# peterrum/dealii-multigrid

Measured on AMD Instinct MI355X. Metric: DoF/s per V-cycle, 3D octant p=4, higher is better.
Workload: dtype f64; 1 GPU; 3D octant (GeometryType quadrant) HMG-global p=4 FP64, NRefGlobal=8, SmootherDegree=3, coarse solver direct, f=1, zero Dirichlet (BASELINE.json configs[2]); n_dofs=137199985, n_cells=2127189, n_levels=9, parallelism=1 GPU, chebyshev_start_vector=deal.II's (i mod 11) - mean on the local numbering, fused_transfer_bricks=33509

## Files before the change

### dealii_multigrid_amd/csrc/kernels_apply.hpp

```cpp
#pragma once
#include "kernels_common.hpp"

namespace mgamd
{
#ifdef MGAMD_KERNEL_DEBUG
#define MGAMD_STAMP(k)                         \
  if (args.stamps && tid == 0)                 \
    args.stamps[(size_t)block * 8 + (k)] = wall_clock64();
#define MGAMD_ABLATED(bit) (args.ablate & (bit))
#else
#define MGAMD_STAMP(k)
#define MGAMD_ABLATED(bit) false
#endif

  template <typename T, int P>
  __device__ __forceinline__ void
  interior_diag_terms(const Mats<P, T> &mats, const int t, T &s_K, T &s_M)
  {
    const int tt[3] = {t % P, (t / P) % P, t / (P * P)};
    T         m[3], k[3];
#pragma unroll
    for (int d = 0; d < 3; ++d)
      {
        T dm = T(0), dk = T(0);
// ... 1174 lines not shown
#pragma unroll
          for (int a = 0; a <= P; ++a)
            {
              dM[c * P + a] += T(args.m.M[a * (P + 1) + a]);
              dK[c * P + a] += T(args.m.K[a * (P + 1) + a]);
            }
        const T sh3 = T(args.sigma) * q * h;
        T       mx = T(0), kx = T(0), my = T(0), ky = T(0);
#pragma unroll
        for (int i = 0; i < G::N; ++i)
          {
            if (i == u)
              {
                mx = dM[i];
                kx = dK[i];
              }
            if (i == v)
              {
                my = dM[i];
                ky = dK[i];
              }
          }
#pragma unroll
        for (int i = 0; i < G::N; ++i)
          bufD[sl * G::N3 + (i * G::N + v) * G::N + u] = h * (kx * my * dM[i] + mx * ky * dM[i] + mx * my * dK[i]) + sh3 * (mx * my * dM[i]);
      }
    __syncthreads();
    if (B == 1)
      {
        const bool any_hanging = __syncthreads_or((int)(mask >> 3)) != 0;
        if (any_hanging)
          for (int j = 0; j < G::N3; ++j)
            {
              for (int idx = tid; idx < G::SPW * G::N3; idx += G::BLOCK)
                bufA[idx] = (idx % G::N3) == j ? T(1) : T(0);
              __syncthreads();
              hanging_passes<T, P>(bufA, args.m, sl, u, v, act, mask, false);
              lattice_sweeps<T, P, B, G::BLOCK>(bufA, bufB, args.m, tid, nslots, args.g.h + slot0, NoHook(), false, args.sigma, args.g.q + slot0);
              hanging_passes<T, P>(bufA, args.m, sl, u, v, act, mask, true);
              if (act && ln == 0 && (mask >> 3))
                bufD[sl * G::N3 + j] = bufA[sl * G::N3 + j];
              __syncthreads();
            }
      }
    if constexpr (brick_may_be_constrained(B, CONSTR))
      {
        uint32_t fm = 0;
        if (args.g.fmask != nullptr && tid < nslots)
          fm = args.g.fmask[slot0 + tid];
        const bool any_family = __syncthreads_or((int)(fm != 0)) != 0;
        if (any_family)
          for (int s = 0; s < G::N_SHELL; ++s)
            {
              const int j = args.g.shell_pos[s];
              for (int idx = tid; idx < G::SPW * G::N3; idx += G::BLOCK)
                bufA[idx] = (idx % G::N3) == j ? T(1) : T(0);
              __syncthreads();
              brick_constraint_passes<T, P, B, G::BLOCK>(bufA, args.m, tid, nslots, args.g.fmask + slot0, false);
              lattice_sweeps<T, P, B, G::BLOCK>(bufA, bufB, args.m, tid, nslots, args.g.h + slot0, NoHook(), false, args.sigma, args.g.q + slot0);
              brick_constraint_passes<T, P, B, G::BLOCK>(bufA, args.m, tid, nslots, args.g.fmask + slot0, true);
              if (act && ln == 0 && args.g.fmask[slot0 + sl])
                bufD[sl * G::N3 + j] = bufA[sl * G::N3 + j];
              __syncthreads();
            }
      }
    if (G::N_INT > 0)
      for (int idx = tid; idx < nslots * G::N_INT; idx += G::BLOCK)
        {
          const int sl2 = idx / (G::N_INT > 0 ? G::N_INT : 1), i = idx % (G::N_INT > 0 ? G::N_INT : 1);
          const int x = i % (G::NI > 0 ? G::NI : 1), y = (i / (G::NI > 0 ? G::NI : 1)) % (G::NI > 0 ? G::NI : 1),
                    z = i / (G::NI > 0 ? G::NI * G::NI : 1);
          const T d = bufD[sl2 * G::N3 + ((z + 1) * G::N + (y + 1)) * G::N + x + 1];
          apply_epilogue<T, MODE_INVDIAG>(args.epi, args.g.interior_base[slot0 + sl2] + i, d);
        }
    for (int idx = tid; idx < nslots * G::N_SHELL; idx += G::BLOCK)
      {
        const int      sl2 = idx / G::N_SHELL, s = idx % G::N_SHELL;
        const uint32_t gi  = args.g.shell_idx[(size_t)(slot0 + sl2) * G::N_SHELL + s];
        if (gi < args.scatter_limit)
          atomic_add(&args.tail_acc[gi - args.n_interior], bufD[sl2 * G::N3 + args.g.shell_pos[s]]);
      }
  }

  template <typename T, int MODE_>
  __global__ void
  __launch_bounds__(256) tail_kernel(T *__restrict__ tail_acc, uint32_t n_interior, uint32_t n_tail, uint32_t n_rest, Epilogue<T> epi)
  {
    constexpr int  MODE   = base_mode(MODE_);
    constexpr bool FUSE_P = MODE_ == MODE_CHEB_PROLONGATE;
    constexpr int  U      = 4;
    const uint32_t total  = n_tail + n_rest;
    const uint32_t stride = gridDim.x * blockDim.x;
    __shared__ T   dtable[256];
    const bool     coded = is_cheb(MODE) && epi.dinv_code != nullptr;
    if (coded)
      {
        dtable[threadIdx.x] = epi.dinv_table[threadIdx.x];
        __syncthreads();
      }
    for (uint32_t i0 = blockIdx.x * blockDim.x + threadIdx.x; i0 < total; i0 += U * stride)
      {
        T ax[U], xv[U], xo[U], bv[U], dv[U];
#pragma unroll
        for (int u = 0; u < U; ++u)
          {
            const uint32_t i  = i0 + u * stride;
            const uint32_t gi = n_interior + i;
            ax[u] = xv[u] = xo[u] = bv[u] = dv[u] = T(0);
            if (i < total)
              {
                if (MODE != MODE_INVDIAG && MODE != MODE_CHEB_FIRST && MODE != MODE_MASS && (is_cheb(MODE) || i >= n_tail))
                  {
                    if (FUSE_P && i < n_tail && NT_LOAD(&epi.xs_flag[i]))
                      {
                        xv[u] = NT_LOAD(&epi.xs[gi]);
                        epi.x_inout[gi] = xv[u];
                      }
                    else
                      xv[u] = NT_LOAD(&epi.x[gi]);
                  }
                ax[u] = i < n_tail ? tail_acc[i] : xv[u];
                if (MODE == MODE_RESIDUAL || is_cheb(MODE))
                  bv[u] = NT_LOAD(&epi.b[gi]);
                if (is_cheb(MODE))
                  {
                    if (MODE == MODE_CHEB && epi.xold)
                      xo[u] = NT_LOAD(&epi.xold[gi]);
                    if (coded)
                      {
                        const uint32_t c = NT_LOAD(&epi.dinv_code[i]);
                        dv[u]            = c != 255u ? dtable[c] : epi.dinv[gi];
                      }
                    else
                      dv[u] = epi.dinv[gi];
                  }
              }
          }
#pragma unroll
        for (int u = 0; u < U; ++u)
          {
            const uint32_t i  = i0 + u * stride;
            const uint32_t gi = n_interior + i;
            if (i < total)
              {
                if (i < n_tail)
                  NT_STORE(T(0), &tail_acc[i]);
                if (MODE == MODE_CHEB_FIRST || MODE == MODE_CHEB_SECOND)
                  {
                    const T x1 = epi.c0 * dv[u] * bv[u];
                    if (MODE == MODE_CHEB_FIRST)
                      {
                        xv[u] = x1;
                        if (i >= n_tail)
                          ax[u] = x1;
                      }
                    else
                      xo[u] = x1;
                  }
                if (MODE == MODE_VMULT || MODE == MODE_MASS)
                  NT_STORE(ax[u], &epi.out[gi]);
                else if (MODE == MODE_RESIDUAL)
                  NT_STORE(bv[u] - ax[u], &epi.out[gi]);
                else if (is_cheb(MODE))
                  {
                    const T r = xv[u] + epi.f1 * (xv[u] - xo[u]) + epi.f2 * dv[u] * (bv[u] - ax[u]);
                    if (MODE_ == MODE_CHEB)
                      store_result(epi, gi, r);
                    else
                      NT_STORE(r, &epi.out[gi]);
                  }
                else
                  epi.out[gi] = (i < n_tail && fabs((double)ax[u]) > 1.0e-10) ? T(1) / ax[u] : T(1);
              }
          }
      }
  }

}
```

### dealii_multigrid_amd/csrc/level_operator.hpp

```cpp
#pragma once
#include "runtime.hpp"
#include "kernels.hpp"

#include <cmath>
#include <cstring>
#include <map>
#include <mutex>
#include <type_traits>
#include <unordered_map>

namespace mgamd
{
  inline int
  grid_for(size_t n)
  {
    size_t g = (n + 255) / 256;
    if (g > 2048)
      g = 2048;
    if (g < 1)
      g = 1;
    return (int)g;
  }

  template <typename T>
// ... 127 lines not shown
      if (any)
        h_cell.upload(g.h);
    }
    const double *
    scale(bool mass_pass) const
    {
      return mass_pass && h_cell.p ? h_cell.p : h.p;
    }
    SlotGroupDev
    view(bool mass_pass) const
    {
      return SlotGroupDev{interior_base.p, shell_idx.p, mask.p, scale(mass_pass), shell_pos.p, (uint32_t)n_slots, fmask.p, q.p};
    }
    SlotGroupDev
    view(size_t begin, size_t end, bool mass_pass) const
    {
      const size_t n_shell = (size_t)N * N * N - (size_t)(N - 2) * (N - 2) * (N - 2);
      return SlotGroupDev{interior_base.p + begin, shell_idx.p + begin * n_shell, mask.p + begin, scale(mass_pass) + begin, shell_pos.p,
                          (uint32_t)(end - begin), fmask.p ? fmask.p + begin : nullptr, q.p + begin};
    }
    DBuf<uint32_t> uniq_ptr, uniq_idx;
    DBuf<uint16_t> loc;
    uint32_t       max_uniq = 0;
    bool
    has_clusters() const
    {
      return uniq_ptr.p != nullptr;
    }
    CellClusterDev
    cluster_view(bool mass_pass) const
    {
      return CellClusterDev{uniq_ptr.p, uniq_idx.p, loc.p, mask.p, scale(mass_pass), (uint32_t)n_slots, max_uniq, q.p};
    }
    size_t
    cluster_lds_bytes() const
    {
      return 2 * (size_t)std::max<uint32_t>(max_uniq, 1) * sizeof(T);
    }
    void
    build_clusters(const SlotGroup &g)
    {
      const size_t          ns = g.n_slots(), ncl = (ns + CLUSTER_CELLS - 1) / CLUSTER_CELLS;
      std::vector<uint32_t> ptr(ncl + 1, 0), idx;
      std::vector<uint16_t> l(ns * 8, 0xFFFFu);
      std::vector<uint32_t> tmp;
      for (size_t c = 0; c < ncl; ++c)
        {
          const size_t s0 = c * CLUSTER_CELLS, s1 = std::min(ns, s0 + CLUSTER_CELLS);
          tmp.clear();
          for (size_t sl = s0; sl < s1; ++sl)
            for (int s = 0; s < 8; ++s)
              if (g.shell_idx[sl * 8 + s] != INVALID_DOF)
                tmp.push_back(g.shell_idx[sl * 8 + s]);
          std::sort(tmp.begin(), tmp.end());
          tmp.erase(std::unique(tmp.begin(), tmp.end()), tmp.end());
          for (size_t sl = s0; sl < s1; ++sl)
            for (int s = 0; s < 8; ++s)
              {
                const uint32_t gi = g.shell_idx[sl * 8 + s];
                if (gi != INVALID_DOF)
                  l[sl * 8 + g.shell_pos[s]] = (uint16_t)(std::lower_bound(tmp.begin(), tmp.end(), gi) - tmp.begin());
              }
          idx.insert(idx.end(), tmp.begin(), tmp.end());
          ptr[c + 1] = (uint32_t)idx.size();
          max_uniq   = std::max<uint32_t>(max_uniq, (uint32_t)tmp.size());
        }
      if (idx.empty())
        idx.push_back(0);
      uniq_ptr.upload(ptr);
      uniq_idx.upload(idx);
      loc.upload(l);
    }
  };

  template <typename T>
  struct FusedTransferHost
  {
    int                 group = -1;
    const uint32_t     *flags = nullptr;
    const uint32_t     *coarse_idx = nullptr;
    uint32_t            nc3 = 0;
    std::vector<double> E;
    const uint8_t      *tail_flags = nullptr;
    T *coarse = nullptr, *scratch = nullptr, *x_inout = nullptr;
  };
  constexpr bool
  fused_transfer_supported(int p)
  {
    return persistent_brick(p) != 0;
  }

  template <typename T>
  struct LevelOperator : LevelOperatorBase
  {
    int                                       p = 1;
    std::vector<std::unique_ptr<GroupDev<T>>> groups;
    DBuf<T>                                   tail_acc;
    DBuf<uint8_t>                             dinv_code;
    DBuf<T>                                   dinv_table;
    const T                                  *dinv_coded = nullptr;
    int                                       dominant_B = 0;
    uint32_t                                  ablate = 0;
    DBuf<unsigned long long>                  stamps;
    int                                       stamp_mode = -1;
    bool                                      halo_overlap = true;

    struct HaloDev
    {
      DBuf<uint32_t> pack_idx, sh_tail, sh_ptr;
      DBuf<int32_t>  sh_src, sh_owner_src;
      DBuf<T>        send, recv;
    };
    std::unique_ptr<HaloDev> halo;

    enum class LaunchKind
    {
      LATTICE,
      LATTICE_CONSTRAINED,
      BRICK_PAIR,
      BRICKS_AND_CELLS,
      BRICKS_AND_CLUSTERS,
      CLUSTERS
    };
    struct LaunchStep
    {
      LaunchKind   kind;
      GroupDev<T> *g, *partner;
      size_t       begin, end;
    };
    struct LaunchPlan
    {
      std::vector<LaunchStep> ordinary, diagonal;
      std::vector<LaunchStep> halo_slots, interior_slots;
    } plan;

    LevelOperator(Ctx *c, const mgamd_dofs *dofs, std::shared_ptr<Comm> cm)
    {
      ctx    = c;
      type   = (int)sizeof(T);
      tables = dofs->tables;
      tria   = dofs->tria;
      p      = tables->p;
      sigma  = tables->sigma;
      if (tables->ls_level && sigma != 0.0)
        throw std::invalid_argument("level operator: mass coefficient " + std::to_string(sigma) +
                                    " on a local-smoothing level: not implemented (refinement-edge matrices have no mass term)");
      if (cm && dofs->halo)
        {
          comm      = cm;
          halo_plan = dofs->halo;
          halo      = std::make_unique<HaloDev>();
          halo->pack_idx.upload(halo_plan->pack_idx);
          halo->sh_tail.upload(halo_plan->sh_tail);
          halo->sh_ptr.upload(halo_plan->sh_ptr);
          halo->sh_src.upload(halo_plan->sh_src);
          halo->sh_owner_src.upload(halo_plan->sh_owner_src);
          halo->send.alloc(std::max<size_t>(halo_plan->pack_idx.size(), 1));
          halo->recv.alloc(std::max<size_t>(halo_plan->pack_idx.size(), 1));
        }
      size_t best = 0;
      for (const SlotGroup &g : tables->groups)
        {
          auto d     = std::make_unique<GroupDev<T>>();
          d->B           = g.B;
          d->N           = g.N;
          d->constrained = g.constrained_group;
// ... 295 lines not shown
    void
    launch_bricks_and_cells(hipStream_t st, const ApplyArgs<T, P> &a, const GroupDev<T> &g1)
    {
      using G2 = Geo<P, 2>;
      SmallSlotsArgs<T, P> sa;
      sa.a           = a;
      sa.g_cells     = g1.view(MODE == MODE_MASS);
      sa.n_wg_bricks = (uint32_t)((a.g.n_slots + G2::SPW - 1) / G2::SPW);
      using GW = Geo<P, 1, 64>;
      const uint32_t n_w        = (uint32_t)((g1.n_slots + GW::SPW - 1) / GW::SPW);
      const uint32_t n_wg_cells = (n_w + CELL_WAVES - 1) / CELL_WAVES;
      constexpr size_t lds      = small_slots_lds_bytes<T, P>();
      static_assert(lds <= 64 * 1024, "above the default dynamic-LDS limit the launch has to go through launch_lds");
      hipLaunchKernelGGL((a.sigma == 0.0 || MODE == MODE_MASS ? lattice_apply_small_kernel<T, P, MODE, false> :
                                                                 lattice_apply_small_kernel<T, P, MODE, true>),
                         sa.n_wg_bricks + n_wg_cells, 256, lds, st, sa);
      HIP_CHECK(hipGetLastError());
    }

    template <int P, int MODE_>
    void
    launch_step(hipStream_t st, ApplyArgs<T, P> &a, const LaunchStep &s, bool diag, const FusedTransferHost<T> *fused, bool stamp = false)
    {
      constexpr int MODE = base_mode(MODE_);
      using K            = LaunchKind;
      GroupDev<T> *g     = s.g;
      a.g                = g->view(s.begin, s.end, MODE == MODE_MASS);
      a.stamps           = nullptr;
      if constexpr (MODE_ != MODE)
        if (fused && fused->group >= 0 && g == groups[fused->group].get())
          return launch_fused<P, MODE_>(st, a, s.begin, s.partner, *fused);
      if (stamp && stamps.p && s.kind != K::BRICK_PAIR && g->B == dominant_B && !g->constrained && MODE == stamp_mode)
        a.stamps = stamps.p;
      bool done = false;
      switch (s.kind)
        {
          case K::LATTICE:
            if (!dispatch_brick_size<P, 1, 2, 4, 8, 16>(g->B, [&](auto B) { launch_lattice<T, P, B(), MODE>(ctx, st, a, diag); }))
              throw std::runtime_error("unsupported brick size");
            break;
          case K::LATTICE_CONSTRAINED:
            if constexpr (P == 1)
              done = dispatch_brick_size<P, 4, 8, 16>(g->B, [&](auto B) { launch_lattice<T, P, B(), MODE, true>(ctx, st, a, diag); });
            if (!done)
              throw std::runtime_error("constrained bricks of this size/degree are not instantiated");
            break;
          case K::BRICK_PAIR:
            if constexpr (P == 1)
              done = dispatch_brick_size<P, 8, 16>(g->B, [&](auto B) { launch_pair<P, B(), MODE>(st, a, s.partner); });
            if (!done)
              throw std::runtime_error("brick pair launch: size not instantiated");
            break;
          case K::BRICKS_AND_CELLS:
            if constexpr (P >= 2)
              launch_bricks_and_cells<P, MODE>(st, a, *s.partner);
            break;
          case K::BRICKS_AND_CLUSTERS:
            if constexpr (P == 1)
              launch_bricks_and_clusters<MODE>(st, a, *s.partner);
            break;
          case K::CLUSTERS:
            launch_clusters<P, MODE == MODE_MASS>(st, *g, a, MODE == MODE_CHEB_FIRST, s.begin, s.end);
            break;
        }
    }

    template <int MODE>
    void
    launch_tail(hipStream_t st, uint32_t begin, uint32_t end, bool with_rest, const Epilogue<T> &epi_in, bool diag)
    {
      const uint32_t n_rest = with_rest ? tables->n_dofs - tables->n_interior - end : 0;
      const uint32_t n_t    = end - begin + n_rest;
      if (!n_t)
        return;
      Epilogue<T> epi = epi_in;
      if (epi.dinv_code)
        epi.dinv_code += begin;
      if (diag)
        hipLaunchKernelGGL((tail_kernel<T, MODE_INVDIAG>), grid_for(n_t), 256, 0, st, tail_acc.p + begin, tables->n_interior + begin, end - begin,
                           n_rest, epi);
      else
        hipLaunchKernelGGL((tail_kernel<T, MODE>), grid_for(n_t), 256, 0, st, tail_acc.p + begin, tables->n_interior + begin, end - begin, n_rest,
                           epi);
      HIP_CHECK(hipGetLastError());
    }

    enum EdgeMode
    {
      EDGE_OUT  = 0,
      EDGE_ROWS = 1,
      EDGE_IN   = 2
    };

    template <int P, int MODE>
    void
    apply_P(const T *src, const Epilogue<T> &epi, bool diag, double words, int edge_mode, const FusedTransferHost<T> *fused);

    template <int MODE>
    void
    apply(const T *src, const Epilogue<T> &epi, bool diag = false, double words = 0, int edge_mode = EDGE_OUT,
          const FusedTransferHost<T> *fused = nullptr)
    {
      constexpr bool FUSED_MODE = MODE != base_mode(MODE);
      if (FUSED_MODE && (!fused || fused->group < 0 || !fused_transfer_supported(p)))
        throw std::runtime_error("fused transfer pass without fused tables");
      auto run = [&](auto P) {
        if constexpr (!FUSED_MODE || fused_transfer_supported(P()))
          apply_P<P(), MODE>(src, epi, diag, words, edge_mode, fused);
      };
      if (!dispatch_degree(p, run))
        throw std::runtime_error("degree not instantiated");
    }

    void
    vmult_raw(T *dst, const T *src)
    {
      Epilogue<T> e{dst, src, nullptr, nullptr, nullptr, T(0), T(0), T(0)};
      apply<MODE_VMULT>(src, e);
    }
    void
    residual_raw(T *t, const T *b, const T *x)
    {
      Epilogue<T> e{t, x, nullptr, b, nullptr, T(0), T(0), T(0)};
      apply<MODE_RESIDUAL>(x, e, false, 0, tables->n_edge ? EDGE_IN : EDGE_OUT);
    }
    void
    vmult_interface_down(mgamd_vec &dst, const mgamd_vec &src) override
    {
      if (dst.n != n_dofs() || src.n != n_dofs() || dst.data == src.data)
        throw std::invalid_argument("vmult_interface_down: bad vectors");
      Epilogue<T> e{dst.as<T>(), src.as<T>(), nullptr, nullptr, nullptr, T(0), T(0), T(0)};
      apply<MODE_VMULT>(src.as<T>(), e, false, 0, tables->n_edge ? EDGE_IN : EDGE_OUT);
    }
    void
    interface_up_raw(T *dst, const T *src, T *tmp)
    {
      const size_t n = n_dofs(), first_edge = (size_t)tables->n_interior + tables->n_tail;
      HIP_CHECK(hipMemsetAsync(tmp, 0, n * sizeof(T), ctx->stream));
      if (tables->n_edge)
        HIP_CHECK(hipMemcpyAsync(tmp + first_edge, src + first_edge, (size_t)tables->n_edge * sizeof(T), hipMemcpyDeviceToDevice, ctx->stream));
      Epilogue<T> e{dst, tmp, nullptr, nullptr, nullptr, T(0), T(0), T(0)};
      apply<MODE_VMULT>(tmp, e, false, 0, EDGE_IN);
    }
    void
    vmult_interface_up(mgamd_vec &dst, const mgamd_vec &src) override
    {
      if (dst.n != n_dofs() || src.n != n_dofs() || dst.data == src.data)
        throw std::invalid_argument("vmult_interface_up: bad vectors");
      DBuf<T> tmp;
      tmp.alloc(n_dofs());
      interface_up_raw(dst.as<T>(), src.as<T>(), tmp.p);
      ctx->sync();
    }
    void
    build_dinv_codes(const T *dinv)
    {
      dinv_coded = nullptr;
      if (getenv("MGAMD_NO_DINV_CODES"))
        return;
      const size_t n0 = tables->n_interior, n = (size_t)n_dofs() - n0;
      if (n < 4096)
        return;
      std::vector<T> h(n);
      ctx->sync();
      HIP_CHECK(hipMemcpy(h.data(), dinv + n0, n * sizeof(T), hipMemcpyDeviceToHost));
      using Bits = typename std::conditional<sizeof(T) == 8, uint64_t, uint32_t>::type;
// ... 124 lines not shown
```

### dealii_multigrid_amd/csrc/level_operator_apply.hpp

```cpp
#pragma once
#include "level_operator.hpp"

namespace mgamd
{
  template <typename T>
  template <int P, int MODE>
  void
  LevelOperator<T>::apply_P(const T *src, const Epilogue<T> &epi, bool diag, double words, int edge_mode, const FusedTransferHost<T> *fused)
  {
    ApplyArgs<T, P> a;
    const uint32_t  first_edge = tables->n_interior + tables->n_tail;
    a.gather_limit  = first_edge + (edge_mode == EDGE_IN ? tables->n_edge : 0);
    a.scatter_limit = first_edge + (edge_mode != EDGE_OUT ? tables->n_edge : 0);
    const uint32_t tail_end = tables->n_tail + (edge_mode != EDGE_OUT ? tables->n_edge : 0);
    a.m          = mats<P>();
    a.src        = src;
    a.tail_acc   = tail_acc.p;
    a.n_interior = tables->n_interior;
    a.ablate     = ablate;
    a.stamps     = nullptr;
    a.epi        = epi;
    a.sigma      = sigma;
    if (!diag && !plan.interior_slots.empty())
      {
        for (const LaunchStep &s : plan.halo_slots)
          launch_step<P, MODE>(ctx->stream, a, s, false, fused);
        ctx->order_after(ctx->side, ctx->stream);
        exchange_add_raw(tail_acc.p, ctx->side);
        for (const LaunchStep &s : plan.interior_slots)
          launch_step<P, MODE>(ctx->stream, a, s, false, fused);
        ctx->order_after(ctx->stream, ctx->side);
        launch_tail<MODE>(ctx->stream, 0, tail_end, true, epi, diag);
        return;
      }
    const hipStream_t main = ctx->stream;
    auto prof_begin = [&](const GroupDev<T> &g) {
      const bool prof = ctx->profile && !diag && MODE == MODE_CHEB && !g.constrained && g.B == (ctx->prof_brick ? ctx->prof_brick : dominant_B);
      if (prof)
        {
          if (ctx->prof_used == ctx->prof_events.size())
            {
              hipEvent_t e0, e1;
              HIP_CHECK(hipEventCreate(&e0));
              HIP_CHECK(hipEventCreate(&e1));
              ctx->prof_events.push_back({e0, e1});
            }
          HIP_CHECK(hipEventRecord(ctx->prof_events[ctx->prof_used].first, main));
        }
      return prof;
    };
    auto prof_end = [&](const GroupDev<T> &g, size_t n_slots) {
      HIP_CHECK(hipEventRecord(ctx->prof_events[ctx->prof_used].second, main));
      ++ctx->prof_used;
      const bool   closed_dinv = P == 1 || persistent_lattice(g.N);
      const double w_interior  = words - (closed_dinv ? 1.0 : 0.0);
      const double n1 = (double)(g.N - 1), n2 = (double)(g.N - 2);
      ctx->prof_bytes += sizeof(T) * (double)n_slots * (words * n2 * n2 * n2 + 2.0 * (n1 * n1 * n1 - n2 * n2 * n2));
      ctx->prof_bytes_moved += sizeof(T) * (double)n_slots * (w_interior * n2 * n2 * n2 + 2.0 * (n1 * n1 * n1 - n2 * n2 * n2));
    };
    for (const LaunchStep &s : diag ? plan.diagonal : plan.ordinary)
      {
        const bool prof = prof_begin(*s.g);
        launch_step<P, MODE>(main, a, s, diag, fused, !diag);
        if (prof)
          prof_end(*s.g, s.g->n_slots);
      }
    if (halo)
      exchange_add_raw(tail_acc.p);
    launch_tail<MODE>(main, 0, tail_end, true, epi, diag);
  }

}
```

### dealii_multigrid_amd/csrc/runtime.hip

```cpp
#include "runtime.hpp"
#include "level_operator.hpp"
#include "amg.hpp"
#include "amg_shard.hpp"

#include <chrono>
#include <cmath>
#include <mutex>
#include <set>
#include <unordered_map>
#include <cstring>
#include <type_traits>

namespace mgamd
{
  Ctx::Ctx(int dev)
    : device(dev)
  {
    int        count = 0;
    hipError_t e     = hipGetDeviceCount(&count);
    if (e != hipSuccess || count == 0)
      throw NoDeviceError("no HIP device available: this library has no CPU fallback");
    if (dev < 0 || dev >= count)
      throw std::invalid_argument("device index out of range");
    HIP_CHECK(hipSetDevice(dev));
// ... 501 lines not shown
    {
      if (dst.n != lop->n_dofs() || src.n != lop->n_dofs() || dst.data == src.data)
        throw std::invalid_argument("PreconditionChebyshev::step: bad vectors");
      T *res = step_raw(dst.as<T>(), tmp.p, src.as<T>());
      if (res != dst.as<T>())
        hipLaunchKernelGGL((vec_copy_kernel<T, T>), grid_for(dst.n), 256, 0, lop->ctx->stream, dst.as<T>(), res, dst.n);
    }
  };

  ChebyshevBase *
  make_chebyshev(LevelOperatorBase *op, unsigned degree, double smoothing_range, unsigned eig_cg_n_iterations)
  {
    if (degree < 1)
      throw std::invalid_argument("SmootherDegree must be >= 1");
    if (op->type == MGAMD_F64)
      return new Chebyshev<double>(static_cast<LevelOperator<double> *>(op), degree, smoothing_range, eig_cg_n_iterations);
    return new Chebyshev<float>(static_cast<LevelOperator<float> *>(op), degree, smoothing_range, eig_cg_n_iterations);
  }

  template <typename T>
  struct Transfer2 : Transfer2Base
  {
    struct GroupD
    {
      int                 kind = 0, nf = 2;
      size_t              n_patches = 0;
      DBuf<uint32_t>      coarse_idx, fine_idx, fine_idx_restrict;
      DBuf<uint16_t>      coarse_mask;
      std::vector<double> E;
      DBuf<uint32_t> p1_uniq_ptr, p1_uniq_idx, p1_fine_t, p1_fine_t_restrict;
      DBuf<uint16_t> p1_loc;
      uint32_t       p1_max_uniq = 0;
      void
      build_p1(const std::vector<uint32_t> &cidx, const std::vector<uint32_t> &fidx, const std::vector<uint32_t> *fidx_restrict)
      {
        const size_t          np = n_patches, nwg = (np + PATCH_P1_BLOCK - 1) / PATCH_P1_BLOCK;
        std::vector<uint32_t> ptr(nwg + 1, 0), idx, tmp;
        std::vector<uint16_t> l(np * 8, 0xFFFFu);
        for (size_t w = 0; w < nwg; ++w)
          {
            const size_t a = w * PATCH_P1_BLOCK, b = std::min(np, a + PATCH_P1_BLOCK);
            tmp.clear();
            for (size_t i = a * 8; i < b * 8; ++i)
              if (cidx[i] != INVALID_DOF)
                tmp.push_back(cidx[i]);
            std::sort(tmp.begin(), tmp.end());
            tmp.erase(std::unique(tmp.begin(), tmp.end()), tmp.end());
            for (size_t i = a * 8; i < b * 8; ++i)
              if (cidx[i] != INVALID_DOF)
                l[i] = (uint16_t)(std::lower_bound(tmp.begin(), tmp.end(), cidx[i]) - tmp.begin());
            idx.insert(idx.end(), tmp.begin(), tmp.end());
            ptr[w + 1]  = (uint32_t)idx.size();
            p1_max_uniq = std::max<uint32_t>(p1_max_uniq, (uint32_t)tmp.size());
          }
        if (idx.empty())
          idx.push_back(0);
        auto transpose = [&](const std::vector<uint32_t> &f) {
          std::vector<uint32_t> t(f.size());
          for (size_t q = 0; q < np; ++q)
            for (int k = 0; k < 27; ++k)
              t[(size_t)k * np + q] = f[q * 27 + k];
          return t;
        };
        p1_uniq_ptr.upload(ptr);
        p1_uniq_idx.upload(idx);
        p1_loc.upload(l);
        p1_fine_t.upload(transpose(fidx));
        if (fidx_restrict)
          p1_fine_t_restrict.upload(transpose(*fidx_restrict));
      }
    };
    struct BrickD
    {
      int            B = 2, fine_group = 0;
      size_t         n_bricks = 0;
      size_t         n_unfused = 0;
      bool           fused = false;
      DBuf<uint32_t> slot, coarse_idx, own_shell, own_shell_restrict;
    };
    FusedTransferHost<T> fused;
    DBuf<uint32_t>       fused_flags;
    DBuf<uint32_t>       fused_coarse_idx;
    DBuf<uint8_t>        fused_tail_flags;
    size_t               n_fused_bricks = 0;
    bool
    fused_ready() const
    {
      return fused.group >= 0 && n_fused_bricks > 0;
    }
    uint64_t
    n_fused_bricks_total() const override
    {
      return fused_ready() ? n_fused_bricks : 0;
    }
    GroupD                               grp[3];
    std::vector<std::unique_ptr<BrickD>> bricks;
    LevelOperator<T>                    *fop = nullptr, *cop = nullptr;
    int                                  pc = 1, pf = 1;
    Ctx                                 *ctx = nullptr;
    FE1D                                 fec;

    Transfer2(LevelOperator<T> *f, LevelOperator<T> *c)
      : fec(c->tables->p)
    {
      fine   = f;
      coarse = c;
      fop    = f;
      cop    = c;
      ctx    = f->ctx;
      int fuse_group = -1;
      if (!getenv("MGAMD_NO_FUSED_TRANSFER") && f->tables->tria != c->tables->tria && f->tables->p == c->tables->p &&
          !f->tables->ls_level && !c->tables->ls_level && fused_transfer_supported(f->tables->p))
        for (size_t gi = 0; gi < f->tables->groups.size(); ++gi)
          {
            const SlotGroup &g = f->tables->groups[gi];
            if (persistent_lattice(g.N) && !g.constrained_group && g.n_slots() > 0)
              fuse_group = (int)gi;
          }
      TransferTables tt(*f->tables, *c->tables, true, fuse_group);
      const uint32_t copy_lo = f->tables->n_interior + f->tables->n_tail_owned, copy_hi = f->tables->n_interior + f->tables->n_tail;
      auto           owned_only = [&](std::vector<uint32_t> v) {
        for (uint32_t &i : v)
          if (i != INVALID_DOF && i >= copy_lo && i < copy_hi)
            i = INVALID_DOF;
        return v;
      };
      for (const BrickTransferGroup &bg : tt.bricks)
        {
          auto d        = std::make_unique<BrickD>();
          d->B          = bg.B;
          d->fine_group = bg.fine_group;
          d->n_bricks   = bg.n_bricks();
          d->n_unfused  = bg.fused ? bg.n_unfused : bg.n_bricks();
          d->fused      = bg.fused;
          if (bg.fused && bg.n_bricks() > bg.n_unfused)
            {
              const SlotGroup &fg  = f->tables->groups[bg.fine_group];
              const size_t     ns  = fg.n_slots(), nsh = (size_t)fg.n_shell, nc3 = (size_t)bg.Nc * bg.Nc * bg.Nc;
              if (2 * ((nsh + 255) / 256) > 15)
                throw std::runtime_error("fused transfer: shell too large for the flag word");
              std::vector<uint32_t> fl(ns * 256, 0);
              std::vector<uint32_t> ci(ns * nc3, INVALID_DOF);
              for (size_t q = bg.n_unfused; q < bg.n_bricks(); ++q)
                {
                  const size_t sl = bg.slot[q];
                  for (size_t t = 0; t < 256; ++t)
                    fl[sl * 256 + t] = 0x8000u;
                  for (size_t t = 0; t < nsh; ++t)
                    fl[sl * 256 + t % 256] |= (uint32_t)(bg.shell_flags[q * nsh + t] & 3u) << (2 * (t / 256));
                  std::copy(bg.coarse_idx.begin() + q * nc3, bg.coarse_idx.begin() + (q + 1) * nc3, ci.begin() + sl * nc3);
                  for (size_t t = 0; t < nc3; ++t)
                    if (bg.coarse_idx[q * nc3 + t] == INVALID_DOF)
                      fl[sl * 256 + t % 256] |= 1u << (16 + t / 256);
                }
              fused_flags.upload(fl);
              fused_coarse_idx.upload(ci);
              fused_tail_flags.upload(tt.tail_owned_by_fused);
              fused.group      = bg.fine_group;
              fused.flags      = fused_flags.p;
              fused.coarse_idx = fused_coarse_idx.p;
              fused.nc3        = (uint32_t)nc3;
              fused.E          = fec.embedding(1, f->tables->p);
              fused.tail_flags = fused_tail_flags.p;
              n_fused_bricks   = bg.n_bricks() - bg.n_unfused;
            }
          d->slot.upload(bg.slot);
          d->coarse_idx.upload(bg.coarse_idx);
          d->own_shell.upload(bg.own_shell);
          if (copy_hi > copy_lo)
            d->own_shell_restrict.upload(owned_only(bg.own_shell));
          bricks.push_back(std::move(d));
        }
      pc = tt.pc;
      pf = tt.pf;
      for (int k = 0; k < 3; ++k)
        {
          grp[k].kind      = k;
          grp[k].nf        = tt.groups[k].nf;
          grp[k].n_patches = tt.groups[k].n_patches();
          if (grp[k].n_patches)
            {
              grp[k].coarse_idx.upload(tt.groups[k].coarse_idx);
              grp[k].coarse_mask.upload(tt.groups[k].coarse_mask);
              grp[k].fine_idx.upload(tt.groups[k].fine_idx);
              if (copy_hi > copy_lo)
                grp[k].fine_idx_restrict.upload(owned_only(tt.groups[k].fine_idx));
              if (k == 1 && tt.pc == 1 && grp[k].nf == 3)
                {
                  if (copy_hi > copy_lo)
                    {
                      const std::vector<uint32_t> fr = owned_only(tt.groups[k].fine_idx);
                      grp[k].build_p1(tt.groups[k].coarse_idx, tt.groups[k].fine_idx, &fr);
                    }
                  else
                    grp[k].build_p1(tt.groups[k].coarse_idx, tt.groups[k].fine_idx, nullptr);
                }
            }
          grp[k].E = fec.embedding(k, pf);
        }
    }

    template <int PC, int NF, bool IDENTITY>
    void
    launch(const GroupD &g, const T *src, T *dst, bool prolongate)
    {
      using G = TransferGeo<PC, NF>;
      TransferArgs<T, PC, NF> a;
      a.coarse_idx  = g.coarse_idx.p;
      a.coarse_mask = g.coarse_mask.p;
      a.fine_idx    = (!prolongate && g.fine_idx_restrict.p) ? g.fine_idx_restrict.p : g.fine_idx.p;
      a.n_patches   = (uint32_t)g.n_patches;
      const int n   = PC + 1;
      for (int i = 0; i < n * n; ++i)
        {
          a.m.M[i] = a.m.K[i] = 0.0;
          a.m.I0[i]           = fec.I[0][i];
          a.m.I1[i]           = fec.I[1][i];
        }
      if ((int)g.E.size() != NF * n)
        throw std::runtime_error("transfer: embedding size mismatch");
      for (int i = 0; i < NF * n; ++i)
        a.E[i] = g.E[i];
      a.src            = src;
      a.dst            = dst;
      const size_t lds = 2 * (size_t)G::SPW * G::NF3 * sizeof(T);
      const int    grid = (int)((g.n_patches + G::SPW - 1) / G::SPW);
      if (prolongate)
        launch_lds(ctx, ctx->stream, prolongate_kernel<T, PC, NF, IDENTITY>, grid, G::BLOCK, lds, a);
      else
        launch_lds(ctx, ctx->stream, restrict_kernel<T, PC, NF, IDENTITY>, grid, G::BLOCK, lds, a);
      HIP_CHECK(hipGetLastError());
    }

    void
    launch_p1(const GroupD &g, const T *src, T *dst, bool prolongate)
    {
      PatchP1Args<T> a;
      a.uniq_ptr    = g.p1_uniq_ptr.p;
      a.uniq_idx    = g.p1_uniq_idx.p;
      a.loc         = g.p1_loc.p;
      a.coarse_mask = g.coarse_mask.p;
      a.fine_idx_t  = (!prolongate && g.p1_fine_t_restrict.p) ? g.p1_fine_t_restrict.p : g.p1_fine_t.p;
      a.n_patches   = (uint32_t)g.n_patches;
      a.max_uniq    = g.p1_max_uniq;
      for (int i = 0; i < 4; ++i)
        {
          a.m.M[i] = a.m.K[i] = 0.0;
// ... 1648 lines not shown
```

### dealii_multigrid_amd/csrc/transfer_tables.hpp

```cpp
#pragma once
#include "level_tables.hpp"

namespace mgamd
{
  struct TransferGroup
  {
    int                   kind = 0, nf = 2;
    std::vector<uint32_t> coarse_idx;
    std::vector<uint16_t> coarse_mask;
    std::vector<uint32_t> fine_idx;
    size_t
    n_patches() const
    {
      return coarse_mask.size();
    }
  };

  struct BrickTransferGroup
  {
    int                   fine_group = 0, B = 2, Nf = 3, Nc = 2;
    std::vector<uint32_t> slot;
    std::vector<uint32_t> coarse_idx;
    std::vector<uint32_t> own_shell;
    static constexpr uint8_t SHELL_OWN = 1, SHELL_OTHER = 2;
// ... 155 lines not shown
            {
              if (pf != pc)
                throw std::runtime_error("transfer: refined cell in a p-transfer");
              kind = 1;
              if (coarse.ls_level && !tf.index.find(cell_key(cc.level + 1, 2 * cc.i, 2 * cc.j, 2 * cc.k)))
                continue;
              bool any_local = false;
              for (int t = 0; t < 8; ++t)
                {
                  const int32_t *f = tf.index.find(cell_key(cc.level + 1, 2 * cc.i + (t & 1), 2 * cc.j + ((t >> 1) & 1), 2 * cc.k + (t >> 2)));
                  if (f && fine.cell_is_local((size_t)*f))
                    any_local = true;
                }
              if (!any_local)
                continue;
            }
          TransferGroup &g = groups[kind];
          g.coarse_mask.push_back(tc.masks[ci]);
          for (int c = 0; c < nc1; ++c)
            for (int b = 0; b < nc1; ++b)
              for (int a = 0; a < nc1; ++a)
                {
                  const int l[3] = {a, b, c};
                  g.coarse_idx.push_back(coarse.cell_node_index(ci, l));
                }
          const int nf = g.nf;
          for (int Z = 0; Z < nf; ++Z)
            for (int Y = 0; Y < nf; ++Y)
              for (int X = 0; X < nf; ++X)
                {
                  uint32_t idx = INVALID_DOF;
                  if (kind == 1)
                    {
                      const int lo[3] = {X > pc ? 1 : 0, Y > pc ? 1 : 0, Z > pc ? 1 : 0};
                      const int hi[3] = {X >= pc ? 1 : 0, Y >= pc ? 1 : 0, Z >= pc ? 1 : 0};
                      for (int cz = lo[2]; cz <= hi[2] && idx == INVALID_DOF; ++cz)
                        for (int cy = lo[1]; cy <= hi[1] && idx == INVALID_DOF; ++cy)
                          for (int cx = lo[0]; cx <= hi[0] && idx == INVALID_DOF; ++cx)
                            {
                              const int32_t *f = tf.index.find(cell_key(cc.level + 1, 2 * cc.i + cx, 2 * cc.j + cy, 2 * cc.k + cz));
                              if (!f)
                                throw std::runtime_error("transfer: fine mesh is not a one-level refinement of the coarse mesh");
                              if (!fine.cell_is_local((size_t)*f))
                                continue;
                              const int l[3] = {X - cx * pc, Y - cy * pc, Z - cz * pc};
                              bool      constrained, corner;
                              uint32_t  v = fine.cell_node_index((size_t)*f, l, &constrained, &corner);
                              if (constrained && !corner)
                                v = INVALID_DOF;
                              idx = v;
                            }
                    }
                  else
                    {
                      const int l[3] = {X, Y, Z};
                      bool      constrained, corner;
                      idx = fine.cell_node_index((size_t)*same, l, &constrained, &corner);
                      if (constrained && !corner)
                        idx = INVALID_DOF;
                    }
                  if (idx != INVALID_DOF)
                    {
                      if (claimed[idx])
                        idx = INVALID_DOF;
                      else
                        claimed[idx] = true;
                    }
                  g.fine_idx.push_back(idx);
                }
        }
      for (BrickTransferGroup &bg : bricks)
        if (bg.fused)
          {
            const SlotGroup        &fg     = fine.groups[bg.fine_group];
            const std::vector<bool> before = claimed;
            bg.shell_flags.assign(bg.n_bricks() * (size_t)fg.n_shell, 0);
            for (size_t q = bg.n_unfused; q < bg.n_bricks(); ++q)
              claim_brick(bg, fg, bg.slot[q], &before, &bg.shell_flags[q * (size_t)fg.n_shell]);
            tail_owned_by_fused.assign(fine.n_tail, 0);
            for (size_t q = bg.n_unfused; q < bg.n_bricks(); ++q)
              for (int t = 0; t < fg.n_shell; ++t)
                if (bg.shell_flags[q * (size_t)fg.n_shell + t] == BrickTransferGroup::SHELL_OWN)
                  tail_owned_by_fused[bg.own_shell[q * (size_t)fg.n_shell + t] - fine.n_interior] = 1;
          }
    }
  };
}

namespace mgamd
{
  inline void
  ls_copy_indices(const LevelTables &global, const LevelTables &lev, int level, std::vector<uint32_t> &gidx, std::vector<uint32_t> &lidx)
  {
    gidx.clear();
    lidx.clear();
    if (global.p != lev.p || !lev.ls_level)
      throw std::invalid_argument("ls_copy_indices: need the active-mesh tables and a local-smoothing level of the same degree");
    const Tria       &tg = *global.tria, &tl = *lev.tria;
    const int         n  = global.p + 1;
    std::vector<bool> seen(lev.n_dofs, false);
    for (size_t gc = 0; gc < tg.cells.size(); ++gc)
      {
        const Cell &c = tg.cells[gc];
        if ((int)c.level != level || !global.cell_is_local(gc))
          continue;
        const int32_t *lc = tl.index.find(cell_key(c));
        if (!lc)
          throw std::runtime_error("ls_copy_indices: active cell missing on its level mesh");
        for (int z = 0; z < n; ++z)
          for (int y = 0; y < n; ++y)
            for (int x = 0; x < n; ++x)
              {
                const int      a[3] = {x, y, z};
                const uint32_t li   = lev.cell_node_index((size_t)*lc, a);
                if (li == INVALID_DOF || li >= lev.first_constrained() || seen[li])
                  continue;
                bool           constrained = false;
                const uint32_t gi          = global.cell_node_index(gc, a, &constrained);
                if (constrained || gi == INVALID_DOF || gi >= global.first_constrained())
                  throw std::runtime_error("ls_copy_indices: a level-interior DoF of an active cell is constrained on the active mesh");
                seen[li] = true;
                gidx.push_back(gi);
                lidx.push_back(li);
              }
      }
  }
}
```

Baseline: 14.95 billion DoF/s.

## Restrict residual-restrict tail epilogue to tail DoFs touched by unfused slots

Adds a host-built list of contiguous tail index runs, limited to shell DoFs of slots not handled by fused transfer bricks. For MODE_RESIDUAL_RESTRICT without halo or edges, a new kernel walks only those runs in 64-wide chunks instead of sweeping the whole tail. The aim is to skip tail rows already owned by the fused transfer, cutting memory traffic in the residual epilogue. The shared row logic is factored into a device helper. Correctness depends on the fused path fully covering the skipped rows, including zeroing tail_acc.

```diff
diff --git a/dealii_multigrid_amd/csrc/kernels_apply.hpp b/dealii_multigrid_amd/csrc/kernels_apply.hpp
--- a/dealii_multigrid_amd/csrc/kernels_apply.hpp
+++ b/dealii_multigrid_amd/csrc/kernels_apply.hpp
@@ -1280,13 +1280,96 @@
       }
   }
 
+  constexpr int TAIL_U = 4;
+  template <typename T, int MODE_>
+  __device__ __forceinline__ void
+  tail_rows(T *__restrict__ tail_acc, const uint32_t n_interior, const uint32_t n_tail, const uint32_t (&row)[TAIL_U], const bool (&live)[TAIL_U],
+            const Epilogue<T> &epi, const T *dtable, const bool coded)
+  {
+    constexpr int  MODE   = base_mode(MODE_);
+    constexpr bool FUSE_P = MODE_ == MODE_CHEB_PROLONGATE;
+    constexpr int  U      = TAIL_U;
+    T ax[U], xv[U], xo[U], bv[U], dv[U];
+#pragma unroll
+    for (int u = 0; u < U; ++u)
+      {
+        const uint32_t i  = row[u];
+        const uint32_t gi = n_interior + i;
+        ax[u] = xv[u] = xo[u] = bv[u] = dv[u] = T(0);
+        if (live[u])
+          {
+            if (MODE != MODE_INVDIAG && MODE != MODE_CHEB_FIRST && MODE != MODE_MASS && (is_cheb(MODE) || i >= n_tail))
+              {
+                if (FUSE_P && i < n_tail && NT_LOAD(&epi.xs_flag[i]))
+                  {
+                    xv[u] = NT_LOAD(&epi.xs[gi]);
+                    epi.x_inout[gi] = xv[u];
+                  }
+                else
+                  xv[u] = NT_LOAD(&epi.x[gi]);
+              }
+            ax[u] = i < n_tail ? tail_acc[i] : xv[u];
+            if (MODE == MODE_RESIDUAL || is_cheb(MODE))
+              bv[u] = NT_LOAD(&epi.b[gi]);
+            if (is_cheb(MODE))
+              {
+                if (MODE == MODE_CHEB && epi.xold)
+                  xo[u] = NT_LOAD(&epi.xold[gi]);
+                if (coded)
+                  {
+                    const uint32_t c = NT_LOAD(&epi.dinv_code[i]);
+                    dv[u]            = c != 255u ? dtable[c] : epi.dinv[gi];
+                  }
+                else
+                  dv[u] = epi.dinv[gi];
+              }
+          }
+      }
+#pragma unroll
+    for (int u = 0; u < U; ++u)
+      {
+        const uint32_t i  = row[u];
+        const uint32_t gi = n_interior + i;
+        if (live[u])
+          {
+            if (i < n_tail)
+              NT_STORE(T(0), &tail_acc[i]);
+            if (MODE == MODE_CHEB_FIRST || MODE == MODE_CHEB_SECOND)
+              {
+                const T x1 = epi.c0 * dv[u] * bv[u];
+                if (MODE == MODE_CHEB_FIRST)
+                  {
+                    xv[u] = x1;
+                    if (i >= n_tail)
+                      ax[u] = x1;
+                  }
+                else
+                  xo[u] = x1;
+              }
+            if (MODE == MODE_VMULT || MODE == MODE_MASS)
+              NT_STORE(ax[u], &epi.out[gi]);
+            else if (MODE == MODE_RESIDUAL)
+              NT_STORE(bv[u] - ax[u], &epi.out[gi]);
+            else if (is_cheb(MODE))
+              {
+                const T r = xv[u] + epi.f1 * (xv[u] - xo[u]) + epi.f2 * dv[u] * (bv[u] - ax[u]);
+                if (MODE_ == MODE_CHEB)
+                  store_result(epi, gi, r);
+                else
+                  NT_STORE(r, &epi.out[gi]);
+              }
+            else
+              epi.out[gi] = (i < n_tail && fabs((double)ax[u]) > 1.0e-10) ? T(1) / ax[u] : T(1);
+          }
+      }
+  }
+
   template <typename T, int MODE_>
   __global__ void
   __launch_bounds__(256) tail_kernel(T *__restrict__ tail_acc, uint32_t n_interior, uint32_t n_tail, uint32_t n_rest, Epilogue<T> epi)
   {
     constexpr int  MODE   = base_mode(MODE_);
-    constexpr bool FUSE_P = MODE_ == MODE_CHEB_PROLONGATE;
-    constexpr int  U      = 4;
+    constexpr int  U      = TAIL_U;
     const uint32_t total  = n_tail + n_rest;
     const uint32_t stride = gridDim.x * blockDim.x;
     __shared__ T   dtable[256];
@@ -1298,80 +1381,44 @@
       }
     for (uint32_t i0 = blockIdx.x * blockDim.x + threadIdx.x; i0 < total; i0 += U * stride)
       {
-        T ax[U], xv[U], xo[U], bv[U], dv[U];
+        uint32_t row[U];
+        bool     live[U];
 #pragma unroll
         for (int u = 0; u < U; ++u)
           {
-            const uint32_t i  = i0 + u * stride;
-            const uint32_t gi = n_interior + i;
-            ax[u] = xv[u] = xo[u] = bv[u] = dv[u] = T(0);
-            if (i < total)
-              {
-                if (MODE != MODE_INVDIAG && MODE != MODE_CHEB_FIRST && MODE != MODE_MASS && (is_cheb(MODE) || i >= n_tail))
-                  {
-                    if (FUSE_P && i < n_tail && NT_LOAD(&epi.xs_flag[i]))
-                      {
-                        xv[u] = NT_LOAD(&epi.xs[gi]);
-                        epi.x_inout[gi] = xv[u];
-                      }
-                    else
-                      xv[u] = NT_LOAD(&epi.x[gi]);
-                  }
-                ax[u] = i < n_tail ? tail_acc[i] : xv[u];
-                if (MODE == MODE_RESIDUAL || is_cheb(MODE))
-                  bv[u] = NT_LOAD(&epi.b[gi]);
-                if (is_cheb(MODE))
-                  {
-                    if (MODE == MODE_CHEB && epi.xold)
-                      xo[u] = NT_LOAD(&epi.xold[gi]);
-                    if (coded)
-                      {
-                        const uint32_t c = NT_LOAD(&epi.dinv_code[i]);
-                        dv[u]            = c != 255u ? dtable[c] : epi.dinv[gi];
-                      }
-                    else
-                      dv[u] = epi.dinv[gi];
-                  }
-              }
-          }
-#pragma unroll
-        for (int u = 0; u < U; ++u)
-          {
-            const uint32_t i  = i0 + u * stride;
-            const uint32_t gi = n_interior + i;
-            if (i < total)
-              {
-                if (i < n_tail)
-                  NT_STORE(T(0), &tail_acc[i]);
-                if (MODE == MODE_CHEB_FIRST || MODE == MODE_CHEB_SECOND)
-                  {
-                    const T x1 = epi.c0 * dv[u] * bv[u];
-                    if (MODE == MODE_CHEB_FIRST)
-                      {
-                        xv[u] = x1;
-                        if (i >= n_tail)
-                          ax[u] = x1;
-                      }
-                    else
-                      xo[u] = x1;
-                  }
-                if (MODE == MODE_VMULT || MODE == MODE_MASS)
-                  NT_STORE(ax[u], &epi.out[gi]);
-                else if (MODE == MODE_RESIDUAL)
-                  NT_STORE(bv[u] - ax[u], &epi.out[gi]);
-                else if (is_cheb(MODE))
-                  {
-                    const T r = xv[u] + epi.f1 * (xv[u] - xo[u]) + epi.f2 * dv[u] * (bv[u] - ax[u]);
-                    if (MODE_ == MODE_CHEB)
-                      store_result(epi, gi, r);
-                    else
-                      NT_STORE(r, &epi.out[gi]);
-                  }
-                else
-                  epi.out[gi] = (i < n_tail && fabs((double)ax[u]) > 1.0e-10) ? T(1) / ax[u] : T(1);
-              }
-          }
-      }
+            row[u]  = i0 + u * stride;
+            live[u] = row[u] < total;
+          }
+        tail_rows<T, MODE_>(tail_acc, n_interior, n_tail, row, live, epi, dtable, coded);
+      }
+  }
+
+  constexpr uint32_t TAIL_CHUNK = 64;
+  template <typename T, int MODE_>
+  __global__ void
+  __launch_bounds__(256) tail_runs_kernel(T *__restrict__ tail_acc, uint32_t n_interior, uint32_t n_tail, const uint32_t *__restrict__ chunks,
+                                          uint32_t n_chunks, Epilogue<T> epi)
+  {
+    constexpr int MODE = base_mode(MODE_);
+    constexpr int U    = TAIL_U;
+    static_assert(!is_cheb(MODE), "run-walking epilogue: modes without the D^-1 code table");
+    const uint32_t c0   = (blockIdx.x * (256 / TAIL_CHUNK) + threadIdx.x / TAIL_CHUNK) * U;
+    const uint32_t lane = threadIdx.x % TAIL_CHUNK;
+    uint32_t       row[U];
+    bool           live[U];
+#pragma unroll
+    for (int u = 0; u < U; ++u)
+      {
+        const uint32_t c = c0 + u;
+        row[u]           = 0;
+        live[u]          = false;
+        if (c < n_chunks)
+          {
+            row[u]  = chunks[2 * c] + lane;
+            live[u] = row[u] < chunks[2 * c + 1];
+          }
+      }
+    tail_rows<T, MODE_>(tail_acc, n_interior, n_tail, row, live, epi, nullptr, false);
   }
 
 }
diff --git a/dealii_multigrid_amd/csrc/level_operator.hpp b/dealii_multigrid_amd/csrc/level_operator.hpp
--- a/dealii_multigrid_amd/csrc/level_operator.hpp
+++ b/dealii_multigrid_amd/csrc/level_operator.hpp
@@ -233,6 +233,8 @@
     uint32_t            nc3 = 0;
     std::vector<double> E;
     const uint8_t      *tail_flags = nullptr;
+    const uint32_t     *tail_chunks   = nullptr;
+    uint32_t            n_tail_chunks = 0;
     T *coarse = nullptr, *scratch = nullptr, *x_inout = nullptr;
   };
   constexpr bool
@@ -694,6 +696,18 @@
       else
         hipLaunchKernelGGL((tail_kernel<T, MODE>), grid_for(n_t), 256, 0, st, tail_acc.p + begin, tables->n_interior + begin, end - begin, n_rest,
                            epi);
+      HIP_CHECK(hipGetLastError());
+    }
+
+    template <int MODE>
+    void
+    launch_tail_runs(hipStream_t st, const uint32_t *chunks, uint32_t n_chunks, const Epilogue<T> &epi)
+    {
+      if (!n_chunks)
+        return;
+      constexpr uint32_t per_wg = 256 / TAIL_CHUNK * TAIL_U;
+      hipLaunchKernelGGL((tail_runs_kernel<T, MODE>), (n_chunks + per_wg - 1) / per_wg, 256, 0, st, tail_acc.p, tables->n_interior, tables->n_tail,
+                         chunks, n_chunks, epi);
       HIP_CHECK(hipGetLastError());
     }
 
diff --git a/dealii_multigrid_amd/csrc/level_operator_apply.hpp b/dealii_multigrid_amd/csrc/level_operator_apply.hpp
--- a/dealii_multigrid_amd/csrc/level_operator_apply.hpp
+++ b/dealii_multigrid_amd/csrc/level_operator_apply.hpp
@@ -67,6 +67,9 @@
       }
     if (halo)
       exchange_add_raw(tail_acc.p);
+    if constexpr (MODE == MODE_RESIDUAL_RESTRICT)
+      if (!diag && !halo && !tables->n_edge && fused && fused->tail_chunks)
+        return launch_tail_runs<MODE>(main, fused->tail_chunks, fused->n_tail_chunks, epi);
     launch_tail<MODE>(main, 0, tail_end, true, epi, diag);
   }
 
diff --git a/dealii_multigrid_amd/csrc/runtime.hip b/dealii_multigrid_amd/csrc/runtime.hip
--- a/dealii_multigrid_amd/csrc/runtime.hip
+++ b/dealii_multigrid_amd/csrc/runtime.hip
@@ -607,6 +607,7 @@
     DBuf<uint32_t>       fused_flags;
     DBuf<uint32_t>       fused_coarse_idx;
     DBuf<uint8_t>        fused_tail_flags;
+    DBuf<uint32_t>       fused_tail_chunks;
     size_t               n_fused_bricks = 0;
     bool
     fused_ready() const
@@ -688,6 +689,26 @@
               fused.E          = fec.embedding(1, f->tables->p);
               fused.tail_flags = fused_tail_flags.p;
               n_fused_bricks   = bg.n_bricks() - bg.n_unfused;
+              if (!f->halo && !f->tables->n_edge)
+                {
+                  std::vector<uint32_t> runs = tt.residual_tail_runs, chunks;
+                  if (f->tables->n_dofs > f->tables->n_interior + f->tables->n_tail)
+                    {
+                      runs.push_back(f->tables->n_tail);
+                      runs.push_back(f->tables->n_dofs - f->tables->n_interior);
+                    }
+                  for (size_t k = 0; k + 1 < runs.size(); k += 2)
+                    for (uint32_t b0 = runs[k]; b0 < runs[k + 1]; b0 += TAIL_CHUNK)
+                      {
+                        chunks.push_back(b0);
+                        chunks.push_back(std::min(runs[k + 1], b0 + TAIL_CHUNK));
+                      }
+                  fused.n_tail_chunks = (uint32_t)(chunks.size() / 2);
+                  if (chunks.empty())
+                    chunks.push_back(0);
+                  fused_tail_chunks.upload(chunks);
+                  fused.tail_chunks = fused_tail_chunks.p;
+                }
             }
           d->slot.upload(bg.slot);
           d->coarse_idx.upload(bg.coarse_idx);
diff --git a/dealii_multigrid_amd/csrc/transfer_tables.hpp b/dealii_multigrid_amd/csrc/transfer_tables.hpp
--- a/dealii_multigrid_amd/csrc/transfer_tables.hpp
+++ b/dealii_multigrid_amd/csrc/transfer_tables.hpp
@@ -261,7 +261,57 @@
               for (int t = 0; t < fg.n_shell; ++t)
                 if (bg.shell_flags[q * (size_t)fg.n_shell + t] == BrickTransferGroup::SHELL_OWN)
                   tail_owned_by_fused[bg.own_shell[q * (size_t)fg.n_shell + t] - fine.n_interior] = 1;
+            if (bg.n_bricks() > bg.n_unfused)
+              build_residual_tail_runs(fine, bg);
           }
+    }
+
+    std::vector<uint32_t> residual_tail_runs;
+    size_t
+    residual_tail_size() const
+    {
+      size_t n = 0;
+      for (size_t k = 0; k + 1 < residual_tail_runs.size(); k += 2)
+        n += residual_tail_runs[k + 1] - residual_tail_runs[k];
+      return n;
+    }
+
+  private:
+    void
+    build_residual_tail_runs(const LevelTables &fine, const BrickTransferGroup &fused_bricks)
+    {
+      std::vector<bool> in_s(fine.n_tail, false);
+      for (size_t gi = 0; gi < fine.groups.size(); ++gi)
+        {
+          const SlotGroup  &g = fine.groups[gi];
+          std::vector<bool> slot_fused(g.n_slots(), false);
+          if ((int)gi == fused_bricks.fine_group)
+            for (size_t q = fused_bricks.n_unfused; q < fused_bricks.n_bricks(); ++q)
+              slot_fused[fused_bricks.slot[q]] = true;
+          for (size_t s = 0; s < g.n_slots(); ++s)
+            if (!slot_fused[s])
+              for (int t = 0; t < g.n_shell; ++t)
+                {
+                  const uint32_t idx = g.shell_idx[s * (size_t)g.n_shell + t];
+                  if (idx != INVALID_DOF && idx >= fine.n_interior && idx - fine.n_interior < fine.n_tail)
+                    in_s[idx - fine.n_interior] = true;
+                }
+        }
+      residual_tail_runs.clear();
+      for (uint32_t i = 0; i < fine.n_tail;)
+        {
+          if (!in_s[i])
+            {
+              ++i;
+              continue;
+            }
+          uint32_t e = i;
+          while (e < fine.n_tail && in_s[e])
+            ++e;
+          residual_tail_runs.push_back(i);
+          residual_tail_runs.push_back(e);
+          i = e;
+        }
     }
   };
 }
```

Result: no change. 15.20 billion DoF/s (median of 6 runs) (+1.6%).
